# lyuchenyang/Macaw-LLM

Measured on AMD Instinct MI355X. Metric: multimodal samples/sec (img+audio+128 tok) fwd+bwd at 1/2/4/8 MI355X, higher is better.
Workload: dtype bf16; 1 GPU; BASELINE cfg 3: CLIP-ViT-L/14 + Whisper-base + LLaMA-7B, image + 30 s audio + 128-token text (S=144); fwd+bwd+fused AdamW, encoders frozen as run_clm_llms.py:390-393, alignment-attention dropout on; global_batch=32, per_gpu_batch=32, seq_len=144, parallelism=dp1: 20 flat buckets, 13476 MiB of parameters, local (one fused AdamW launch), step_launch=eager, kernel by kernel, grad_weight_side_stream=off (engine.DW_SIDE auto), setup_steps=1, activation_checkpointing=False

## Files before the change

macaw_llm_amd/build.py:

```python
from __future__ import annotations

import hashlib
import os
import shutil
import subprocess
import sys
from concurrent.futures import ThreadPoolExecutor
from pathlib import Path

PKG = Path(__file__).resolve().parent
CSRC = PKG / "csrc"
OBJ = PKG / "csrc" / "_obj"
LIB = PKG / "libmacaw_hip.so"
ARCH = "gfx950"
EXPERIMENTS = bool(os.environ.get("MK_EXPERIMENTS"))
SOURCES = ["gemm.hip", "gemm_v7.hip", *(["gemm_v8.hip"] if EXPERIMENTS else []), "gemm_v9.hip", "norm.hip",
           "elementwise.hip", "softmax.hip", "attention.hip", "decode.hip", "decode_fp8.hip", "sample.hip", "preprocess.hip", "lora.hip"]
FLAGS = ["-O3", "-std=c++17", "-fPIC", f"--offload-arch={ARCH}", "-fno-gpu-rdc", *os.environ.get("MK_EXTRA_FLAGS", "").split(),
         *(["-DMK_WITH_V8", "-DMK_WITH_FWD4X64"] if EXPERIMENTS else []), "-Wno-unused-result"]


FILE_FLAGS = {"gemm_v8.hip": ["-mllvm", "-pragma-unroll-threshold=1000000"],
              "gemm_v9.hip": ["-mllvm", "-pragma-unroll-threshold=1000000"]}


def _hipcc() -> str:
    for cand in (os.environ.get("HIPCC"), shutil.which("hipcc"), "/opt/rocm/bin/hipcc"):
        if cand and Path(cand).exists():
            return cand
    raise RuntimeError("hipcc not found: cannot build libmacaw_hip.so")


def _digest(paths) -> str:
    h = hashlib.sha256()
    for p in sorted(paths):
        h.update(p.name.encode())
        h.update(p.read_bytes())
    h.update(" ".join(FLAGS).encode())
    h.update(repr(sorted(FILE_FLAGS.items())).encode())
    return h.hexdigest()


def build(force: bool = False, verbose: bool = True) -> Path:
    srcs = [CSRC / s for s in SOURCES]
    deps = srcs + [CSRC / "common.h", CSRC / "gemm_common.h", PKG.parent / "include" / "macaw_hip.h",
                   *sorted(CSRC.glob("*.inc"))]
    stamp = OBJ / "stamp.txt"
    dig = _digest(deps)
    if not force and LIB.exists() and stamp.exists() and stamp.read_text() == dig:
        return LIB
    OBJ.mkdir(parents=True, exist_ok=True)
    hipcc = _hipcc()

    def compile_one(src: Path) -> Path:
        obj = OBJ / (src.stem + ".o")
        cmd = [hipcc, *FLAGS, *FILE_FLAGS.get(src.name, []), "-c", str(src), "-o", str(obj)]
        r = subprocess.run(cmd, capture_output=True, text=True)
        if r.returncode != 0:
            raise RuntimeError(f"hipcc failed for {src.name}:\n{r.stderr[-4000:]}")
        return obj

    with ThreadPoolExecutor(max_workers=min(8, len(srcs))) as ex:
        objs = list(ex.map(compile_one, srcs))
    cmd = [hipcc, "-shared", "-fPIC", f"--offload-arch={ARCH}", "-o", str(LIB), *map(str, objs)]
    r = subprocess.run(cmd, capture_output=True, text=True)
    if r.returncode != 0:
        raise RuntimeError(f"link failed:\n{r.stderr[-4000:]}")
    stamp.write_text(dig)
    if verbose:
        print(f"[macaw_llm_amd.build] built {LIB} ({LIB.stat().st_size/1e6:.1f} MB)", file=sys.stderr)
    return LIB


if __name__ == "__main__":
    build(force="--force" in sys.argv)
```

macaw_llm_amd/csrc/gemm.hip:

```cpp
#include "common.h"
#include "../../include/macaw_hip.h"
#include "gemm_common.h"
#include <cstdio>
#include <algorithm>
#include <cstdlib>
#include <utility>
#include <vector>

namespace {
using namespace mkg;

constexpr int BM = 128, BN = 128, BK = 64;
#ifndef MK_GEMM_DEFAULT_CFG
#define MK_GEMM_DEFAULT_CFG 5
#endif
constexpr int TILE_BYTES = 128 * 64 * 2;
}

#define MK_E16_T bf16
#define MK_E16_NS e_bf16
#include "gemm_impl.inc"
#undef MK_E16_T
#undef MK_E16_NS
#define MK_E16_T _Float16
#define MK_E16_NS e_f16
#define gemm_bf16_kernel gemm_f16_kernel
#define gemm_bf16_v2_kernel gemm_f16_v2_kernel
#define gemm_fp8_v2_kernel gemm_fp8_v2_kernel_unused
#include "gemm_impl.inc"
#undef gemm_bf16_kernel
#undef gemm_bf16_v2_kernel
#undef gemm_fp8_v2_kernel
#undef MK_E16_T
#undef MK_E16_NS

namespace {
using namespace mkg;

constexpr int FBM = 64, FBN = 64, FBK = 16, FPAD = 4;

template <bool RED_MAJOR>
MK_DEV void f32_tile_load(const float* base, long ld, int row0, int k0, int R, int K,
                          float (*lds)[FBM + FPAD]) {
  const int t = threadIdx.x;
  if constexpr (!RED_MAJOR) {
    const int row = t >> 2, kq = (t & 3) * 4;
    const int gr = row0 + row;
#pragma unroll
    for (int j = 0; j < 4; ++j) {
      const int gk = k0 + kq + j;
      lds[kq + j][row] = (gr < R && gk < K) ? base[(long)gr * ld + gk] : 0.f;
    }
  } else {
    const int kr = t >> 4, mq = (t & 15) * 4;
    const int gk = k0 + kr;
#pragma unroll
    for (int j = 0; j < 4; ++j) {
      const int gr = row0 + mq + j;
      lds[kr][mq + j] = (gr < R && gk < K) ? base[(long)gk * ld + gr] : 0.f;
    }
  }
}

template <bool A_RED, bool B_RED>
__global__ __launch_bounds__(256) void gemm_f32_kernel(GemmArgs g) {
  __shared__ float As[FBK][FBM + FPAD];
  __shared__ float Bs[FBK][FBN + FPAD];
  int tm, tn;
  tile_coords(blockIdx.x, g.tiles_m, g.tiles_n, tm, tn);
  const int z = blockIdx.z, z1 = z / g.nb2, z2 = z - z1 * g.nb2;
  const float* A = reinterpret_cast<const float*>(g.A) + z1 * g.sA1 + z2 * g.sA2;
  const float* B = reinterpret_cast<const float*>(g.B) + z1 * g.sB1 + z2 * g.sB2;
  float* C = reinterpret_cast<float*>(g.C) + z1 * g.sC1 + z2 * g.sC2;
  const float* Rp = g.R ? reinterpret_cast<const float*>(g.R) + z1 * g.sR1 + z2 * g.sR2 : nullptr;
  const int m0 = tm * FBM, n0 = tn * FBN;
  const int tid = threadIdx.x, l = tid & 63, w = tid >> 6;
  const int wm0 = (w >> 1) * 32, wn0 = (w & 1) * 32;
  f32x4 acc[2][2];
#pragma unroll
  for (int i = 0; i < 2; ++i)
#pragma unroll
    for (int j = 0; j < 2; ++j) acc[i][j] = f32x4{0.f, 0.f, 0.f, 0.f};

  for (int k0 = 0; k0 < g.K; k0 += FBK) {
    f32_tile_load<A_RED>(A, g.lda, m0, k0, g.M, g.K, As);
    f32_tile_load<B_RED>(B, g.ldb, n0, k0, g.N, g.K, Bs);
    __syncthreads();
#pragma unroll
    for (int ks = 0; ks < 4; ++ks) {
      const int kk = ks * 4 + (l >> 4);
      float fm[2], fn[2];
      fm[0] = As[kk][wm0 + (l & 15)];
      fm[1] = As[kk][wm0 + 16 + (l & 15)];
      fn[0] = Bs[kk][wn0 + (l & 15)];
      fn[1] = Bs[kk][wn0 + 16 + (l & 15)];
#pragma unroll
      for (int i = 0; i < 2; ++i)
#pragma unroll
        for (int j = 0; j < 2; ++j)
          acc[i][j] = __builtin_amdgcn_mfma_f32_16x16x4f32(fn[j], fm[i], acc[i][j], 0, 0, 0);
    }
    __syncthreads();
  }
#pragma unroll
  for (int i = 0; i < 2; ++i) {
    const int m = m0 + wm0 + i * 16 + (l & 15);
    if (m >= g.M) continue;
#pragma unroll
    for (int j = 0; j < 2; ++j) {
      const int n = n0 + wn0 + j * 16 + 4 * (l >> 4);
#pragma unroll
      for (int e = 0; e < 4; ++e) {
        if (n + e >= g.N) continue;
        float v = g.alpha * acc[i][j][e];
        if (g.bias_mode == 1) v += reinterpret_cast<const float*>(g.bias)[n + e];
        else if (g.bias_mode == 2) v += reinterpret_cast<const float*>(g.bias)[m];
        v = apply_act(v, g.act);
        if (Rp) v += Rp[(long)m * g.ldr + n + e];
        float* cp = C + (long)m * g.ldc + n + e;
        if (g.accumulate) v += *cp;
        *cp = v;
      }
    }
  }
}

template <typename T>
__global__ __launch_bounds__(256) void transpose_kernel(const T* in, T* out, int rows, int cols,
                                                        long ld_in, long ld_out, long s_in,
                                                        long s_out) {
  __shared__ T tile[64][65];
  in += (long)blockIdx.z * s_in;
  out += (long)blockIdx.z * s_out;
  const int r0 = blockIdx.y * 64, c0 = blockIdx.x * 64;
  const int tx = threadIdx.x & 63, ty = threadIdx.x >> 6;
  for (int i = ty; i < 64; i += 4) {
    const int r = r0 + i, c = c0 + tx;
    if (r < rows && c < cols) tile[i][tx] = in[(long)r * ld_in + c];
  }
  __syncthreads();
  for (int i = ty; i < 64; i += 4) {
    const int c = c0 + i, r = r0 + tx;
    if (r < rows && c < cols) out[(long)c * ld_out + r] = tile[tx][i];
  }
}

bool aligned16(const void* p) { return (reinterpret_cast<uintptr_t>(p) & 15) == 0; }

}


namespace {
struct ProfRec { hipEvent_t a, b; double flops; int kind, M, N, K, nb, layout, cfg; };
bool g_prof_on = false;
std::vector<ProfRec> g_prof;
std::vector<std::pair<hipEvent_t, hipEvent_t>> g_prof_pool;
}

namespace mkp {
bool on() { return g_prof_on; }
int begin(hipStream_t st, int kind, double flops, int M, int N, int K, int nb, int layout, int cfg) {
  if (!g_prof_on) return -1;
  ProfRec rec{};
  if (!g_prof_pool.empty()) { rec.a = g_prof_pool.back().first; rec.b = g_prof_pool.back().second; g_prof_pool.pop_back(); }
  else { (void)hipEventCreate(&rec.a); (void)hipEventCreate(&rec.b); }
  rec.flops = flops; rec.kind = kind; rec.M = M; rec.N = N; rec.K = K; rec.nb = nb; rec.layout = layout; rec.cfg = cfg;
  (void)hipEventRecord(rec.a, st);
  g_prof.push_back(rec);
  return (int)g_prof.size() - 1;
}
void set_cfg(int idx, int cfg) { if (idx >= 0) g_prof[idx].cfg = cfg; }
void end(int idx, hipStream_t st) { if (idx >= 0) (void)hipEventRecord(g_prof[idx].b, st); }
}

extern "C" int mk_prof_begin(void) {
  for (auto& r : g_prof) g_prof_pool.emplace_back(r.a, r.b);
  g_prof.clear();
  g_prof_on = true;
  return MK_OK;
}
extern "C" int mk_prof_sum(int kind, double* total_ms, double* total_flops, int64_t* launches) {
  double ms = 0.0, fl = 0.0;
  int64_t n = 0;
  for (auto& r : g_prof) {
    if (r.kind != kind) continue;
    if (hipEventSynchronize(r.b) != hipSuccess) return MK_ERR_LAUNCH;
    float t = 0.f;
    if (hipEventElapsedTime(&t, r.a, r.b) != hipSuccess) return MK_ERR_LAUNCH;
    ms += t;
    fl += r.flops;
    ++n;
  }
  if (total_ms) *total_ms = ms;
  if (total_flops) *total_flops = fl;
  if (launches) *launches = n;
  return MK_OK;
}
extern "C" int mk_prof_end(double* total_ms, double* total_flops, int64_t* launches) {
  g_prof_on = false;
  return mk_prof_sum(0, total_ms, total_flops, launches);
}

extern "C" int mk_prof_report(const char* path) {
  FILE* f = fopen(path, "w");
  if (!f) return MK_ERR_BAD_ARG;
  struct Agg { int kind, M, N, K, nb, layout, cfg; long n; double ms, fl; };
  std::vector<Agg> aggs;
  for (auto& r : g_prof) {
    if (hipEventSynchronize(r.b) != hipSuccess) { fclose(f); return MK_ERR_LAUNCH; }
    float t = 0.f;
    (void)hipEventElapsedTime(&t, r.a, r.b);
    bool found = false;
    for (auto& a : aggs)
      if (a.kind == r.kind && a.M == r.M && a.N == r.N && a.K == r.K && a.nb == r.nb && a.layout == r.layout && a.cfg == r.cfg) {
        a.n++; a.ms += t; a.fl += r.flops; found = true; break;
      }
    if (!found) aggs.push_back({r.kind, r.M, r.N, r.K, r.nb, r.layout, r.cfg, 1, (double)t, r.flops});
  }
  fprintf(f, "kind,M,N,K,batch,layout,cfg,launches,total_ms,tflops\n");
  for (auto& a : aggs)
    fprintf(f, "%s,%d,%d,%d,%d,%d,%d,%ld,%.4f,%.1f\n", a.kind == 0 ? "gemm" : a.kind == 1 ? "attn_fwd" : a.kind == 2 ? "attn_bwd" : "gemm_fp8",
            a.M, a.N, a.K, a.nb, a.layout, a.cfg, a.n, a.ms, a.ms > 0 ? a.fl / (a.ms * 1e-3) / 1e12 : 0.0);
  fclose(f);
  return MK_OK;
}

namespace { int g_force_cfg = -1; }
namespace {
int skinny32_cfg(int N) {
  const char* e = getenv("MK_GEMM_SKINNY32");
  const int forced = e ? atoi(e) : 0;
  if (forced == 19 || forced == 22) return forced;
  return N >= 8192 ? 22 : 19;
}
}

extern "C" int mk_gemm_set_cfg(int cfg) { g_force_cfg = cfg; return MK_OK; }
extern "C" int mk_gemm_has_cfg(int cfg) {
#ifdef MK_WITH_V8
  if (cfg == 14) return 1;
#endif
  return cfg == 0 || cfg == 5 || cfg == 7 || cfg == 11 || cfg == 15;
}
namespace { int g_plan_cus = 0; }
extern "C" int mk_gemm_set_cus(int n) { const int prev = g_plan_cus; g_plan_cus = n > 0 ? n : 0; return prev; }

namespace mkg {
int launch_v7(const GemmArgs& g, bool a_red, bool b_red, dim3 grid, hipStream_t st, bool fp8, bool f16);
#ifdef MK_WITH_V8
int launch_v8(const GemmArgs& g, bool a_red, bool b_red, dim3 grid, hipStream_t st, bool f16);
#endif
int launch_v9(const GemmArgs& g, bool a_red, bool b_red, dim3 grid, hipStream_t st, bool f16);
int v9_mfma16_layouts();
}

extern "C" int mk_decode_linear(const void* x, int64_t ldx, const void* W, int64_t ldw, void* y,
                                int64_t ldy, const void* residual, int64_t ldr, int32_t M, int32_t N,
                                int32_t K, int32_t prologue, const void* norm_w, float eps,
                                int32_t dtype, void* stream) {
  if (!x || !W || !y || M <= 0 || N <= 0 || K <= 0) return MK_ERR_BAD_ARG;
  if (prologue < 0 || prologue > 2 || (prologue == 1 && !norm_w)) return MK_ERR_BAD_ARG;
  if ((dtype != MK_BF16 && dtype != MK_F16) || M > (prologue ? 16 : 32) || (K % 64) || (ldx % 8) || (ldw % 8) ||
      !aligned16(x) || !aligned16(W) || (prologue == 1 && !aligned16(norm_w)))
    return MK_ERR_UNSUPPORTED;
  GemmArgs g{};
  g.A = x; g.B = W; g.C = y; g.R = residual;
  g.M = M; g.N = N; g.K = K;
  g.lda = ldx; g.ldb = ldw; g.ldc = ldy; g.ldr = ldr;
  g.alpha = 1.f;
  g.pro_w = norm_w; g.pro_eps = eps;
  hipStream_t st = reinterpret_cast<hipStream_t>(stream);
  const bool wide = N <= 16 * 256 && K <= 4096;
  const size_t lds = prologue ? (size_t)M * (K + 8) * 2 : 0;
  if (lds > 40 * 1024) return MK_ERR_UNSUPPORTED;
  const int prof = mkp::begin(st, 0, 2.0 * M * N * K, M, N, K, 1, 0, 17 + 10 * prologue);
  if (M > 16) {
    if (dtype == MK_F16) e_f16::launch_skinny(g, skinny32_cfg(N), N, st);
    else e_bf16::launch_skinny(g, skinny32_cfg(N), N, st);
  } else if (dtype == MK_F16) e_f16::launch_decode_linear(g, N, prologue, wide, lds, st);
  else e_bf16::launch_decode_linear(g, N, prologue, wide, lds, st);
  mkp::end(prof, st);
  return mk_check_launch();
}
namespace {
int pick_cfg(const mk_gemm_desc* d, int nbatch, bool v7_ok, int n_cus) {
  static const bool no_v7 = getenv("MK_GEMM_NO_V7") != nullptr;
  if (!v7_ok || no_v7 || nbatch != 1) return MK_GEMM_DEFAULT_CFG;
  const int layout = (d->a_red_major ? 2 : 0) + (d->b_red_major ? 1 : 0);
  const double nk = (d->K + 63) / 64;
  const long T7 = (long)mk_cdiv(d->M, 256) * mk_cdiv(d->N, 256);
  const long full = T7 / n_cus, R = T7 % n_cus;
  const double a7 = layout == 3 ? 1.53 : layout == 1 ? 1.51 : layout == 2 ? 1.52 : 1.46;
  const double tile7 = nk * a7 + 11.5, sub7 = nk * 0.48 + 7.0;
  double t7 = full * tile7;
  if (R > 0) t7 += (4 * R <= 2 * n_cus) ? (double)mk_cdiv((int)(4 * R), n_cus) * sub7
                                         : nk * a7 * (0.55 + 0.45 * R / n_cus) + 11.5;
  const long T2 = (long)mk_cdiv(d->M, 128) * mk_cdiv(d->N, 128);
  const long slots2 = (long)n_cus * (layout == 3 ? 4 : 2);
  const double tile2 = layout == 3 ? nk * 2.18 + 4.0 : nk * (layout == 0 ? 1.67 : 1.45) + 2.0;
  const double a2 = layout == 3 ? 2.18 : layout == 0 ? 1.67 : 1.45;
  const double nk2 = layout == 3 ? 2 * nk : nk;
  double t2;
  if (T2 < slots2) {
    double sp = (double)(slots2 / T2);
    if (sp > nk2 / 2) sp = nk2 / 2;
    if (sp > 64) sp = 64;
    if (sp < 1) sp = 1;
    const double alone = sp > 1 ? 1.0 : 0.57 + 0.43 * std::min(1.0, std::max(0.0, (double)T2 / n_cus - 1.0));
    t2 = nk / sp * a2 * alone + 2.0 + (sp > 1 ? 4.0 + 1.6 * sp : 0.0);
  } else {
    t2 = (double)T2 / slots2 * tile2;
    if (const long R2 = T2 % slots2) {
      double sp = (double)slots2 / R2;
      if (sp > nk2 / 2) sp = nk2 / 2;
      if (sp > 64) sp = 64;
      t2 += 4.0 + 0.65 * sp;
    }
  }
  if (!(t7 * 0.95 < t2)) return MK_GEMM_DEFAULT_CFG;
  static const int v9_mode = [] { const char* e = getenv("MK_GEMM_V9"); return e ? atoi(e) : 1; }();
  const bool m16 = ((mkg::v9_mfma16_layouts() >> layout) & 1) != 0;
  const bool v9_legal = d->dtype != MK_F32 && d->dtype != MK_FP8 && d->M % 256 == 0 && d->N % 256 == 0 && d->K % 64 == 0 &&
                        full >= 1 && !d->scale_a && !d->scale_b &&
                        d->bias_mode == 0 && d->act == 0 && !d->accumulate && (m16 || !d->R);
  const bool nt16 = m16 && layout == 0 && !(R > 0 && full < 2 && nk < 128);
  if (v9_legal && (v9_mode == 2 || (v9_mode == 1 && (layout == 3 || layout == 1 || nk >= 256 || nt16)))) return 15;
  return 11;
}
}

extern "C" int mk_abi_version(void) { return MK_ABI_VERSION; }

extern "C" int mk_gemm(const mk_gemm_desc* d_in, void* stream) {
  const mk_gemm_desc* d = d_in;
  if (!d || !d->A || !d->B || !d->C) return MK_ERR_BAD_ARG;
  if (d->M <= 0 || d->N <= 0 || d->K <= 0) return MK_ERR_BAD_ARG;
  if (d->nb1 < 1 || d->nb2 < 1) return MK_ERR_BAD_ARG;
  if (d->bias_mode && !d->bias) return MK_ERR_BAD_ARG;
  mk_gemm_desc dd;
  bool fp8 = false;
  if (d->dtype == MK_FP8) {
    if (d->a_red_major || d->b_red_major || (d->K % 128) || (d->lda % 16) || (d->ldb % 16) ||
        (d->sA1 % 16) || (d->sA2 % 16) || (d->sB1 % 16) || (d->sB2 % 16) || !aligned16(d->A) ||
        !aligned16(d->B))
      return MK_ERR_UNSUPPORTED;
    dd = *d;
    dd.K /= 2; dd.lda /= 2; dd.ldb /= 2;
    dd.sA1 /= 2; dd.sA2 /= 2; dd.sB1 /= 2; dd.sB2 /= 2;
    dd.dtype = MK_BF16;
    d = &dd;
    fp8 = true;
  }
  if (d->dtype != MK_F32 && d->dtype != MK_BF16 && d->dtype != MK_F16) return MK_ERR_UNSUPPORTED;
  const bool f16 = d->dtype == MK_F16;
  const bool e16 = d->dtype == MK_BF16 || f16;
  GemmArgs g;
  g.scale_a = d->scale_a; g.scale_b = d->scale_b;
  g.scale_vec = (d->flags & MK_GEMM_SCALE_VEC) ? 1 : 0;
  if (g.scale_vec && (!d->scale_a || !d->scale_b)) return MK_ERR_BAD_ARG;
  if (g.scale_vec && !fp8) return MK_ERR_UNSUPPORTED;
  g.A = d->A; g.B = d->B; g.C = d->C; g.R = d->R; g.bias = d->bias;
  g.M = d->M; g.N = d->N; g.K = d->K;
  g.lda = d->lda; g.ldb = d->ldb; g.ldc = d->ldc; g.ldr = d->ldr;
  g.nb2 = d->nb2;
  g.sA1 = d->sA1; g.sA2 = d->sA2; g.sB1 = d->sB1; g.sB2 = d->sB2;
  g.sC1 = d->sC1; g.sC2 = d->sC2; g.sR1 = d->sR1; g.sR2 = d->sR2;
  g.alpha = d->alpha; g.bias_mode = d->bias_mode; g.act = d->act; g.accumulate = d->accumulate;
  hipStream_t st = reinterpret_cast<hipStream_t>(stream);
  const int nbatch = d->nb1 * d->nb2;
  const int prof = mkp::begin(st, fp8 ? 3 : 0, 2.0 * d->M * d->N * d->K * nbatch * (fp8 ? 2 : 1), d->M, d->N,
                              d->K * (fp8 ? 2 : 1), nbatch, d->a_red_major * 2 + d->b_red_major, -1);
  static const int skinny_max = [] { const char* e = getenv("MK_GEMM_SKINNY_MAX_M"); return e ? atoi(e) : 32; }();
  if (e16 && !fp8 && d->M <= 32 && d->M <= skinny_max && !d->a_red_major && !d->b_red_major && nbatch == 1 &&
      (d->K % 64) == 0 && (d->lda % 8) == 0 && (d->ldb % 8) == 0 && aligned16(d->A) && aligned16(d->B) &&
      !getenv("MK_GEMM_NO_SKINNY")) {
    int sk = d->M <= 16 ? ((d->N <= 16 * 256 && d->K <= 4096) ? 18 : 17) : skinny32_cfg(d->N);
    if ((g_force_cfg == 12 || g_force_cfg == 19 || g_force_cfg == 22) ||
        ((g_force_cfg == 13 || g_force_cfg == 17 || g_force_cfg == 18) && d->M <= 16)) sk = g_force_cfg;
    mkp::set_cfg(prof, sk);
    if (f16) e_f16::launch_skinny(g, sk, d->N, st);
    else e_bf16::launch_skinny(g, sk, d->N, st);
    mkp::end(prof, st);
    return mk_check_launch();
  }
  if (e16) {
    static const int env_cfg0 = [] {
      const char* e = getenv("MK_GEMM_CFG");
      return e ? atoi(e) : -1;
    }();
    const int env_cfg = g_force_cfg >= 0 ? g_force_cfg : env_cfg0;
    const auto fits = [&](bool red, long ld, int rows) {
      const long span = red ? (long)d->K * ld * 2 : ((long)rows * ld + d->K) * 2;
      return span < 0x7fffffffL;
    };
    const long kpad = (d->K + 63) / 64 * 64;
    const bool ktail_a = d->a_red_major || ((d->flags & MK_GEMM_A_KPAD_ZERO) && d->lda >= kpad);
    const bool ktail_b = d->b_red_major || ((d->flags & MK_GEMM_B_KPAD_ZERO) && d->ldb >= kpad);
    const bool v2_ok = aligned16(d->A) && aligned16(d->B) && (d->lda % 8 == 0) && (d->ldb % 8 == 0) &&
                       (d->sA1 % 8 == 0) && (d->sA2 % 8 == 0) && (d->sB1 % 8 == 0) &&
                       (d->sB2 % 8 == 0) &&
                       (d->K % BK == 0 || (ktail_a && ktail_b && d->K > BK)) &&
                       fits(d->a_red_major, d->lda, BM) && fits(d->b_red_major, d->ldb, BN);
    const bool v7_ok = v2_ok && d->K >= 128 && d->M > 128 && d->N > 128 &&
                       fits(d->a_red_major, d->lda, 256) && fits(d->b_red_major, d->ldb, 256);
    static const int dev_cus = [] {
      int dev = 0, cus = 256;
      (void)hipGetDevice(&dev);
      (void)hipDeviceGetAttribute(&cus, hipDeviceAttributeMultiprocessorCount, dev);
      return cus;
    }();
    const int n_cus = (g_plan_cus > 0 && g_plan_cus < dev_cus) ? g_plan_cus : dev_cus;
    int cfg;
    if (env_cfg >= 0) cfg = env_cfg;
    else cfg = pick_cfg(d, nbatch, v7_ok, n_cus);
    if (fp8 && cfg != 11) cfg = 5;
#ifndef MK_WITH_V8
    if (cfg == 14) cfg = 11;
#endif
    if ((cfg == 11 || cfg == 14 || cfg == 15) && !v7_ok) cfg = 5;
    if ((cfg == 14 || cfg == 15) && fp8) cfg = 11;
    if (cfg == 15 && (d->M % 256 != 0 || d->N % 256 != 0 || d->K % 64 != 0 || d->K < 128)) cfg = 11;
    if (cfg == 15 && ((mkg::v9_mfma16_layouts() >> ((d->a_red_major ? 2 : 0) + (d->b_red_major ? 1 : 0))) & 1) &&
        (d->bias_mode != 0 || d->act != 0 || d->accumulate || d->scale_a || d->scale_b))
      cfg = 11;
    if (cfg != 0 && cfg != 5 && cfg != 7 && cfg != 11 && cfg != 14 && cfg != 15) cfg = 5;
    if (cfg >= 5 && !v2_ok) cfg = 0;
    if (fp8 && cfg != 5 && cfg != 11) return MK_ERR_UNSUPPORTED;
    if (cfg == 5 && d->a_red_major && d->b_red_major && !getenv("MK_GEMM_NO_BK32")) cfg = 7;
    const int bkv = cfg == 7 ? 32 : BK;
    mkp::set_cfg(prof, cfg);
    const bool v8 = cfg == 14;
    const bool v9 = cfg == 15;
    const bool t256 = cfg == 11 || v8 || v9;
    const int bm = t256 ? 256 : 128;
    const int bn = t256 ? 256 : BN;
    g.tiles_m = mk_cdiv(d->M, bm);
    g.tiles_n = mk_cdiv(d->N, bn);
    g.a_vec = aligned16(d->A) && (d->lda % 8 == 0) && (d->sA1 % 8 == 0) && (d->sA2 % 8 == 0);
    g.b_vec = aligned16(d->B) && (d->ldb % 8 == 0) && (d->sB1 % 8 == 0) && (d->sB2 % 8 == 0);
    const auto c_aligned = [&](uintptr_t mask, long q) {
      return ((reinterpret_cast<uintptr_t>(d->C) & mask) == 0) && (d->ldc % q == 0) && (d->sC1 % q == 0) &&
             (d->sC2 % q == 0) &&
             (!d->R || (((reinterpret_cast<uintptr_t>(d->R) & mask) == 0) && (d->ldr % q == 0) &&
                        (d->sR1 % q == 0) && (d->sR2 % q == 0)));
    };
    g.c_vec = c_aligned(15, 8) ? 2 : c_aligned(7, 4) ? 1 : 0;
    dim3 grid(g.tiles_m * g.tiles_n, 1, nbatch);
    g.dp_tiles = g.tiles_m * g.tiles_n;
    g.lin_batch = 0;
    g.split = 1;
    g.kt_per_piece = 0;
    g.ws = nullptr;
    g.counters = nullptr;
    g.ablate = 0;
    {
      static const int v9_lds_epi = getenv("MK_V9_LDS_EPI") ? 1 : 0;
      if (cfg == 15 && v9_lds_epi) g.ablate = 9;
    }
    g.tail8 = 0;
    const int slots = n_cus * (t256 ? 1 : (cfg == 7 ? 4 : 2));
    static const bool no_streamk = getenv("MK_GEMM_NO_STREAMK") != nullptr;
    if (t256 && !v8 && !no_streamk) {
      const int T = g.tiles_m * g.tiles_n, R = T % n_cus;
      static const bool no_tail8 = getenv("MK_GEMM_NO_TAIL8") != nullptr;
      if (R > 0 && 8 * R <= n_cus && !d->a_red_major && !no_tail8) {
        g.dp_tiles = T - R;
        g.tail8 = 1;
        grid.x = g.dp_tiles + 8 * R;
      } else if (R > 0 && 4 * R <= 2 * n_cus) {
        g.dp_tiles = T - R;
        grid.x = g.dp_tiles + 4 * R;
      }
    } else if ((cfg == 5 || cfg == 7) && d->ws && !no_streamk) {
      const int T = g.tiles_m * g.tiles_n * nbatch, nkt = (d->K + bkv - 1) / bkv;
      const int R = T % slots;
      int sp = R > 0 ? slots / R : 1;
      if (sp > nkt / 2) sp = nkt / 2;
      if (sp > 64) sp = 64;
      const long need = 4096 + (long)R * sp * (64 * 256) * 4;
      if (R > 0 && sp >= 2 && need <= d->ws_bytes) {
        g.dp_tiles = T - R;
        g.split = sp;
        g.kt_per_piece = (nkt + sp - 1) / sp;
        g.counters = reinterpret_cast<int*>(d->ws);
        g.ws = reinterpret_cast<float*>(reinterpret_cast<char*>(d->ws) + 4096);
        if (R * (int)sizeof(int) > 4096) { g.dp_tiles = T; g.split = 1; }
        else {
          grid.x = g.dp_tiles + R * sp;
          if (nbatch > 1) { g.lin_batch = 1; grid.z = 1; }
        }
      }
    }
    g.walkers = g.dp_tiles;
    if (t256 && !v8 && !v9) {
      static const bool no_walk = getenv("MK_GEMM_NO_WALK") != nullptr;
      if (!no_walk && nbatch == 1 && n_cus % 8 == 0 && g.dp_tiles > n_cus && g.dp_tiles % n_cus == 0) {
        grid.x = n_cus + (grid.x - g.dp_tiles);
        g.walkers = n_cus;
      }
    }
#ifdef MK_WITH_V8
    if (v8) {
      const int rc = mkg::launch_v8(g, d->a_red_major != 0, d->b_red_major != 0, grid, st, f16);
      mkp::end(prof, st);
      return rc;
    }
#endif
    const bool v9_c_ok = !((mkg::v9_mfma16_layouts() >> ((d->a_red_major ? 2 : 0) + (d->b_red_major ? 1 : 0))) & 1) || g.c_vec >= 1;
    if (v9 && g.dp_tiles >= n_cus && v9_c_ok) {
      const int tail_wgs = (int)grid.x - g.walkers;
      dim3 gmain(g.dp_tiles, 1, nbatch);
      static const bool no_walk9 = getenv("MK_GEMM_NO_WALK") != nullptr;
      const bool plain9 = d->bias_mode == 0 && d->act == 0 && !d->R && !d->accumulate && g.c_vec == 2 && !d->scale_a &&
                          !d->scale_b && g.ablate != 9;
      const int lay9 = (d->a_red_major ? 2 : 0) + (d->b_red_major ? 1 : 0);
      const bool regepi9 = plain9 || (((mkg::v9_mfma16_layouts() >> lay9) & 1) && g.c_vec >= 1 && d->bias_mode == 0 && d->act == 0 &&
                                      !d->accumulate && !d->scale_a && !d->scale_b && g.ablate != 9);
      if (!no_walk9 && regepi9 && nbatch == 1 && n_cus % 8 == 0 && g.dp_tiles > n_cus && g.dp_tiles % n_cus == 0)
        gmain.x = n_cus;
      int rc = mkg::launch_v9(g, d->a_red_major != 0, d->b_red_major != 0, gmain, st, f16);
      if (rc == MK_OK && tail_wgs > 0) {
        GemmArgs gt = g;
        gt.walkers = 0;
        rc = mkg::launch_v7(gt, d->a_red_major != 0, d->b_red_major != 0, dim3(tail_wgs, 1, nbatch), st, false, f16);
      }
      mkp::end(prof, st);
      return rc;
    }
    if (t256) {
      if (v9) mkp::set_cfg(prof, 11);
      const int rc = mkg::launch_v7(g, d->a_red_major != 0, d->b_red_major != 0, grid, st, fp8, f16);
      mkp::end(prof, st);
      return rc;
    }
    if (f16) (void)e_f16::launch_tile(g, cfg, d->a_red_major != 0, d->b_red_major != 0, false, grid, st);
    else (void)e_bf16::launch_tile(g, cfg, d->a_red_major != 0, d->b_red_major != 0, fp8, grid, st);
  } else {
    g.tiles_m = mk_cdiv(d->M, FBM);
    g.tiles_n = mk_cdiv(d->N, FBN);
    g.a_vec = g.b_vec = g.c_vec = 0;
    dim3 grid(g.tiles_m * g.tiles_n, 1, nbatch), block(256);
    if (!d->a_red_major && !d->b_red_major)
      MK_LAUNCH((gemm_f32_kernel<false, false>), grid, block, 0, st, g);
    else if (!d->a_red_major && d->b_red_major)
      MK_LAUNCH((gemm_f32_kernel<false, true>), grid, block, 0, st, g);
    else if (d->a_red_major && !d->b_red_major)
      MK_LAUNCH((gemm_f32_kernel<true, false>), grid, block, 0, st, g);
    else
      MK_LAUNCH((gemm_f32_kernel<true, true>), grid, block, 0, st, g);
  }
  mkp::end(prof, st);
  return mk_check_launch();
}

extern "C" int mk_transpose(const void* in, void* out, int32_t rows, int32_t cols, int64_t ld_in,
                            int64_t ld_out, int32_t batch, int64_t s_in, int64_t s_out,
                            int32_t elem_size, void* stream) {
  if (!in || !out || rows <= 0 || cols <= 0 || batch <= 0) return MK_ERR_BAD_ARG;
  dim3 grid(mk_cdiv(cols, 64), mk_cdiv(rows, 64), batch), block(256);
  hipStream_t st = reinterpret_cast<hipStream_t>(stream);
  if (elem_size == 2)
    MK_LAUNCH((transpose_kernel<unsigned short>), grid, block, 0, st,
                       (const unsigned short*)in, (unsigned short*)out, rows, cols, (long)ld_in,
                       (long)ld_out, (long)s_in, (long)s_out);
  else if (elem_size == 4)
    MK_LAUNCH((transpose_kernel<float>), grid, block, 0, st, (const float*)in,
                       (float*)out, rows, cols, (long)ld_in, (long)ld_out, (long)s_in,
                       (long)s_out);
  else
    return MK_ERR_UNSUPPORTED;
  return mk_check_launch();
}
```

Measured before the change: 150.5 samples/s.

## Add 256x128 half-width v7h GEMM kernel with cost-model selection

Adds a new GEMM kernel that uses 256x128 tiles with BK=32, a 3-stage buffer-load-to-LDS pipeline and two workgroups per CU, for non-transposed bf16/f16 layouts. The picker gets a cost model that selects it when the tile count leaves the 256x256 kernels with poor CU fill or too few K iterations. It targets wave-quantization waste on mid-sized GEMMs. The trade-off is lower per-tile arithmetic intensity and risk from a hand-tuned cost model.

```diff
diff --git a/macaw_llm_amd/build.py b/macaw_llm_amd/build.py
--- a/macaw_llm_amd/build.py
+++ b/macaw_llm_amd/build.py
@@ -14,7 +14,7 @@
 LIB = PKG / "libmacaw_hip.so"
 ARCH = "gfx950"
 EXPERIMENTS = bool(os.environ.get("MK_EXPERIMENTS"))
-SOURCES = ["gemm.hip", "gemm_v7.hip", *(["gemm_v8.hip"] if EXPERIMENTS else []), "gemm_v9.hip", "norm.hip",
+SOURCES = ["gemm.hip", "gemm_v7.hip", "gemm_v7h.hip", *(["gemm_v8.hip"] if EXPERIMENTS else []), "gemm_v9.hip", "norm.hip",
            "elementwise.hip", "softmax.hip", "attention.hip", "decode.hip", "decode_fp8.hip", "sample.hip", "preprocess.hip", "lora.hip"]
 FLAGS = ["-O3", "-std=c++17", "-fPIC", f"--offload-arch={ARCH}", "-fno-gpu-rdc", *os.environ.get("MK_EXTRA_FLAGS", "").split(),
          *(["-DMK_WITH_V8", "-DMK_WITH_FWD4X64"] if EXPERIMENTS else []), "-Wno-unused-result"]
diff --git a/macaw_llm_amd/csrc/gemm.hip b/macaw_llm_amd/csrc/gemm.hip
--- a/macaw_llm_amd/csrc/gemm.hip
+++ b/macaw_llm_amd/csrc/gemm.hip
@@ -3,6 +3,7 @@
 #include "gemm_common.h"
 #include <cstdio>
 #include <algorithm>
+#include <cmath>
 #include <cstdlib>
 #include <utility>
 #include <vector>
@@ -240,7 +241,7 @@
 #ifdef MK_WITH_V8
   if (cfg == 14) return 1;
 #endif
-  return cfg == 0 || cfg == 5 || cfg == 7 || cfg == 11 || cfg == 15;
+  return cfg == 0 || cfg == 5 || cfg == 7 || cfg == 11 || cfg == 15 || cfg == 16;
 }
 namespace { int g_plan_cus = 0; }
 extern "C" int mk_gemm_set_cus(int n) { const int prev = g_plan_cus; g_plan_cus = n > 0 ? n : 0; return prev; }
@@ -251,6 +252,7 @@
 int launch_v8(const GemmArgs& g, bool a_red, bool b_red, dim3 grid, hipStream_t st, bool f16);
 #endif
 int launch_v9(const GemmArgs& g, bool a_red, bool b_red, dim3 grid, hipStream_t st, bool f16);
+int launch_v7h(const GemmArgs& g, dim3 grid, hipStream_t st, bool f16);
 int v9_mfma16_layouts();
 }
 
@@ -283,7 +285,7 @@
   return mk_check_launch();
 }
 namespace {
-int pick_cfg(const mk_gemm_desc* d, int nbatch, bool v7_ok, int n_cus) {
+int pick_cfg(const mk_gemm_desc* d, int nbatch, bool v7_ok, bool v7h_ok, int n_cus) {
   static const bool no_v7 = getenv("MK_GEMM_NO_V7") != nullptr;
   if (!v7_ok || no_v7 || nbatch != 1) return MK_GEMM_DEFAULT_CFG;
   const int layout = (d->a_red_major ? 2 : 0) + (d->b_red_major ? 1 : 0);
@@ -317,6 +319,22 @@
       t2 += 4.0 + 0.65 * sp;
     }
   }
+  static const int v7h_mode = [] { const char* e = getenv("MK_GEMM_V7H"); return e ? atoi(e) : 1; }();
+  if (v7h_ok && v7h_mode > 0 && !(full >= 2 && nk >= 64)) {
+    constexpr double V7H_A2 = 2.17, V7H_F2 = 6.5, V7H_L = 3.5, V7H_A1 = 1.38, V7H_F1 = 8.4;
+    const long Th = (long)mk_cdiv(d->M, 256) * mk_cdiv(d->N, 128);
+    const long slots_h = 2L * n_cus;
+    const double alone = nk * V7H_A1 + V7H_F1, round_h = nk * V7H_A2 + V7H_F2;
+    double t7h;
+    if (Th <= n_cus) t7h = alone;
+    else if (Th < slots_h) {
+      const double shared = (double)(Th - n_cus) / n_cus;
+      t7h = (1.0 - shared) * alone + shared * (V7H_L + round_h);
+    } else {
+      t7h = V7H_L + ((double)(Th / slots_h) + std::sqrt((double)(Th % slots_h) / slots_h)) * round_h;
+    }
+    if (v7h_mode == 2 ? nk <= 16 : t7h * 1.07 < std::min(t7, t2)) return 16;
+  }
   if (!(t7 * 0.95 < t2)) return MK_GEMM_DEFAULT_CFG;
   static const int v9_mode = [] { const char* e = getenv("MK_GEMM_V9"); return e ? atoi(e) : 1; }();
   const bool m16 = ((mkg::v9_mfma16_layouts() >> layout) & 1) != 0;
@@ -403,6 +421,8 @@
                        fits(d->a_red_major, d->lda, BM) && fits(d->b_red_major, d->ldb, BN);
     const bool v7_ok = v2_ok && d->K >= 128 && d->M > 128 && d->N > 128 &&
                        fits(d->a_red_major, d->lda, 256) && fits(d->b_red_major, d->ldb, 256);
+    const bool v7h_ok = v7_ok && !fp8 && nbatch == 1 && !d->a_red_major && !d->b_red_major && d->K % 64 == 0 &&
+                        !d->scale_a && !d->scale_b;
     static const int dev_cus = [] {
       int dev = 0, cus = 256;
       (void)hipGetDevice(&dev);
@@ -412,7 +432,8 @@
     const int n_cus = (g_plan_cus > 0 && g_plan_cus < dev_cus) ? g_plan_cus : dev_cus;
     int cfg;
     if (env_cfg >= 0) cfg = env_cfg;
-    else cfg = pick_cfg(d, nbatch, v7_ok, n_cus);
+    else cfg = pick_cfg(d, nbatch, v7_ok, v7h_ok, n_cus);
+    if (cfg == 16 && !v7h_ok) cfg = 11;
     if (fp8 && cfg != 11) cfg = 5;
 #ifndef MK_WITH_V8
     if (cfg == 14) cfg = 11;
@@ -423,7 +444,7 @@
     if (cfg == 15 && ((mkg::v9_mfma16_layouts() >> ((d->a_red_major ? 2 : 0) + (d->b_red_major ? 1 : 0))) & 1) &&
         (d->bias_mode != 0 || d->act != 0 || d->accumulate || d->scale_a || d->scale_b))
       cfg = 11;
-    if (cfg != 0 && cfg != 5 && cfg != 7 && cfg != 11 && cfg != 14 && cfg != 15) cfg = 5;
+    if (cfg != 0 && cfg != 5 && cfg != 7 && cfg != 11 && cfg != 14 && cfg != 15 && cfg != 16) cfg = 5;
     if (cfg >= 5 && !v2_ok) cfg = 0;
     if (fp8 && cfg != 5 && cfg != 11) return MK_ERR_UNSUPPORTED;
     if (cfg == 5 && d->a_red_major && d->b_red_major && !getenv("MK_GEMM_NO_BK32")) cfg = 7;
@@ -431,8 +452,9 @@
     mkp::set_cfg(prof, cfg);
     const bool v8 = cfg == 14;
     const bool v9 = cfg == 15;
+    const bool v7h = cfg == 16;
     const bool t256 = cfg == 11 || v8 || v9;
-    const int bm = t256 ? 256 : 128;
+    const int bm = t256 || v7h ? 256 : 128;
     const int bn = t256 ? 256 : BN;
     g.tiles_m = mk_cdiv(d->M, bm);
     g.tiles_n = mk_cdiv(d->N, bn);
@@ -527,6 +549,11 @@
       mkp::end(prof, st);
       return rc;
     }
+    if (v7h) {
+      const int rc = mkg::launch_v7h(g, grid, st, f16);
+      mkp::end(prof, st);
+      return rc;
+    }
     if (t256) {
       if (v9) mkp::set_cfg(prof, 11);
       const int rc = mkg::launch_v7(g, d->a_red_major != 0, d->b_red_major != 0, grid, st, fp8, f16);
diff --git a/macaw_llm_amd/csrc/gemm_v7h.hip b/macaw_llm_amd/csrc/gemm_v7h.hip
--- /dev/null
+++ b/macaw_llm_amd/csrc/gemm_v7h.hip
@@ -0,0 +1,21 @@
+#include "gemm_common.h"
+#include <type_traits>
+
+#define MK_E16_T bf16
+#define MK_E16_NS e_bf16
+#include "gemm_v7h_impl.inc"
+#undef MK_E16_T
+#undef MK_E16_NS
+#define MK_E16_T _Float16
+#define MK_E16_NS e_f16
+#define gemm_bf16_v7h_kernel gemm_f16_v7h_kernel
+#include "gemm_v7h_impl.inc"
+#undef gemm_bf16_v7h_kernel
+#undef MK_E16_T
+#undef MK_E16_NS
+
+namespace mkg {
+int launch_v7h(const GemmArgs& g, dim3 grid, hipStream_t st, bool f16) {
+  return f16 ? e_f16::launch_v7h(g, grid, st) : e_bf16::launch_v7h(g, grid, st);
+}
+}
diff --git a/macaw_llm_amd/csrc/gemm_v7h_impl.inc b/macaw_llm_amd/csrc/gemm_v7h_impl.inc
--- /dev/null
+++ b/macaw_llm_amd/csrc/gemm_v7h_impl.inc
@@ -0,0 +1,165 @@
+
+
+namespace {
+namespace MK_E16_NS {
+using namespace mkg;
+typedef MK_E16_T e16;
+typedef E16<e16>::x8 e16x8;
+
+constexpr int BMH = 256, BNH = 128, BKH = 32;
+constexpr int A_IMG_H = 128 * 128;
+constexpr int B_IMG_H = 64 * 128;
+constexpr int STAGE_H = A_IMG_H + B_IMG_H;
+constexpr int NSTAGE_H = 3;
+constexpr int LDSH = NSTAGE_H * STAGE_H;
+constexpr int A_PIECES_H = A_IMG_H / 1024 / 4;
+constexpr int B_PIECES_H = B_IMG_H / 1024 / 4;
+
+MK_DEV int v7h_voffset(int row0, int R, long ld, int pair, int p, int l) {
+  const int r = p * 8 + (l >> 3);
+  const int c = (l & 7) ^ ((r >> 1) & 7);
+  const int gr = min(row0 + r + (c >> 2) * pair, R - 1) - row0;
+  return (int)((long)gr * ld * 2 + (c & 3) * 16);
+}
+MK_DEV int v7h_read_offset(int hi, int ks, int l) {
+  const int row = l & 31;
+  const int c = hi * 4 + ks * 2 + (l >> 5);
+  return row * 128 + ((c ^ ((row >> 1) & 7)) << 4);
+}
+
+template <int N>
+MK_DEV void v7h_wait_vm() {
+  if constexpr (N == 0) asm volatile("s_waitcnt vmcnt(0) lgkmcnt(0)" ::: "memory");
+  else asm volatile("s_waitcnt vmcnt(%0) lgkmcnt(0)" ::"n"(N) : "memory");
+}
+
+__global__ __launch_bounds__(256, 2) void gemm_bf16_v7h_kernel(GemmArgs g) {
+  constexpr int FM = 4, FN = 2;
+  __shared__ __attribute__((aligned(16))) char smem[LDSH];
+  int tm, tn;
+  tile_from_index(xcd_remap(blockIdx.x, (int)gridDim.x), g.tiles_m, g.tiles_n, tm, tn, 8);
+  const int m0 = tm * BMH, n0 = tn * BNH;
+  const e16* A = reinterpret_cast<const e16*>(g.A);
+  const e16* B = reinterpret_cast<const e16*>(g.B);
+  e16* C = reinterpret_cast<e16*>(g.C);
+  const e16* Rp = reinterpret_cast<const e16*>(g.R);
+  const int l = threadIdx.x & 63;
+  const int w = __builtin_amdgcn_readfirstlane(threadIdx.x >> 6);
+  const int wr = w >> 1, wc = w & 1;
+  const int wm0 = wr * 128, wn0 = wc * 64;
+  const e16* abase = uniform_ptr(A + (long)m0 * g.lda);
+  const e16* bbase = uniform_ptr(B + (long)n0 * g.ldb);
+  const long a_bytes = ((long)(min(g.M - m0, BMH) - 1) * g.lda + g.K) * 2;
+  const long b_bytes = ((long)(min(g.N - n0, BNH) - 1) * g.ldb + g.K) * 2;
+  const __amdgpu_buffer_rsrc_t rsA = __builtin_amdgcn_make_buffer_rsrc(
+      (void*)abase, 0, (int)min(a_bytes, 0x7fffffffL), 0x00020000);
+  const __amdgpu_buffer_rsrc_t rsB = __builtin_amdgcn_make_buffer_rsrc(
+      (void*)bbase, 0, (int)min(b_bytes, 0x7fffffffL), 0x00020000);
+  int voA[A_PIECES_H], voB[B_PIECES_H];
+#pragma unroll
+  for (int i = 0; i < A_PIECES_H; ++i) voA[i] = v7h_voffset(m0, g.M, g.lda, 128, w + 4 * i, l);
+#pragma unroll
+  for (int i = 0; i < B_PIECES_H; ++i) voB[i] = v7h_voffset(n0, g.N, g.ldb, 64, w + 4 * i, l);
+  int offA[2], offB[2];
+#pragma unroll
+  for (int ks = 0; ks < 2; ++ks) {
+    offA[ks] = v7h_read_offset(wr, ks, l);
+    offB[ks] = A_IMG_H + v7h_read_offset(wc, ks, l);
+  }
+  f32x16 acc[FM][FN];
+#pragma unroll
+  for (int i = 0; i < FM; ++i)
+#pragma unroll
+    for (int j = 0; j < FN; ++j)
+#pragma unroll
+      for (int e = 0; e < 16; ++e) acc[i][j][e] = 0.f;
+
+  const int nk = g.K / BKH;
+  int k_in = 0, st_in = 0;
+  auto piece = [&](int i) {
+    char* dst = smem + st_in * STAGE_H + w * 1024;
+    if (i < A_PIECES_H)
+      __builtin_amdgcn_raw_ptr_buffer_load_lds(
+          rsA, (__attribute__((address_space(3))) void*)(dst + i * 4096), 16, voA[i < A_PIECES_H ? i : 0], k_in, 0, 0);
+    else
+      __builtin_amdgcn_raw_ptr_buffer_load_lds(
+          rsB, (__attribute__((address_space(3))) void*)(dst + A_IMG_H + (i - A_PIECES_H) * 4096), 16,
+          voB[i < A_PIECES_H ? 0 : i - A_PIECES_H], k_in, 0, 0);
+  };
+  auto requested = [&]() {
+    k_in += BKH * 2;
+    st_in = st_in == NSTAGE_H - 1 ? 0 : st_in + 1;
+  };
+#pragma unroll
+  for (int s = 0; s < 2; ++s) {
+#pragma unroll
+    for (int i = 0; i < A_PIECES_H + B_PIECES_H; ++i) piece(i);
+    requested();
+  }
+  int st = 0;
+  auto stage = [&](auto issue_c) {
+    constexpr bool ISSUE = decltype(issue_c)::value;
+    constexpr int NP = A_PIECES_H + B_PIECES_H, NP_EARLY = 2;
+    const char* sa = smem + st * STAGE_H;
+    e16x8 fa[2][FM], fb[2][FN];
+#pragma unroll
+    for (int ks = 0; ks < 2; ++ks) {
+#pragma unroll
+      for (int j = 0; j < FN; ++j) fb[ks][j] = *reinterpret_cast<const e16x8*>(sa + offB[ks] + j * 4096);
+#pragma unroll
+      for (int i = 0; i < FM; ++i) fa[ks][i] = *reinterpret_cast<const e16x8*>(sa + offA[ks] + i * 4096);
+    }
+    __builtin_amdgcn_sched_barrier(0);
+    if constexpr (ISSUE) {
+#pragma unroll
+      for (int i = 0; i < NP_EARLY; ++i) piece(i);
+      __builtin_amdgcn_sched_barrier(0);
+    }
+#pragma unroll
+    for (int ks = 0; ks < 2; ++ks)
+#pragma unroll
+      for (int j = 0; j < FN; ++j)
+#pragma unroll
+        for (int i = 0; i < FM; ++i) {
+          acc[i][j] = E16<e16>::mma32(fb[ks][j], fa[ks][i], acc[i][j]);
+          if constexpr (ISSUE) {
+            const int m = (ks * FN + j) * FM + i;
+            if (m % 2 == 1 && NP_EARLY + m / 2 < NP) {
+              __builtin_amdgcn_sched_barrier(0);
+              piece(NP_EARLY + m / 2);
+              __builtin_amdgcn_sched_barrier(0);
+            }
+          }
+        }
+    if constexpr (ISSUE) requested();
+#pragma unroll
+    for (int i = 0; i < FM; ++i) asm volatile("" : "+v"(acc[i][0]), "+v"(acc[i][1]));
+    st = st == NSTAGE_H - 1 ? 0 : st + 1;
+  };
+  const int nk_issue = nk - 2;
+#pragma unroll 1
+  for (int t = 0; t < nk_issue; ++t) {
+    v7h_wait_vm<A_PIECES_H + B_PIECES_H>();
+    __builtin_amdgcn_sched_barrier(0);
+    __builtin_amdgcn_s_barrier();
+    __builtin_amdgcn_sched_barrier(0);
+    stage(std::true_type{});
+  }
+#pragma unroll 1
+  for (int t = 0; t < 2; ++t) {
+    if (t == 0) v7h_wait_vm<A_PIECES_H + B_PIECES_H>();
+    else v7h_wait_vm<0>();
+    __builtin_amdgcn_sched_barrier(0);
+    __builtin_amdgcn_s_barrier();
+    __builtin_amdgcn_sched_barrier(0);
+    stage(std::false_type{});
+  }
+  wave_epilogue16<false>(acc, g, C, Rp, m0, n0, wm0, wn0, smem);
+}
+
+int launch_v7h(const GemmArgs& g, dim3 grid, hipStream_t st) {
+  MK_LAUNCH(gemm_bf16_v7h_kernel, grid, dim3(256), 0, st, g);
+  return mk_check_launch();
+}
+}
+}
```

Result: no change. 150.5 samples/s, median of 2 (+0.0%).
